# zju3dv/IntrinsicNeRF

Hardware: AMD Instinct MI355X
Metric: rays/sec (64+128 samples/ray) (higher is better)
Workload: dtype f32 (operands split into f16 hi+lo, 3 f16 MFMA products per MAC, fp32 accumulate); 1 GPU; Blender chair 800x800 frame (640000 rays), 64 coarse + 128 importance samples, coarse+fine intrinsic NeRF (D=8, W=256), white_bkgd, eval mode, default-init weights (seeds 0/1) with the density head calibrated so that acc spans (0, 1]; parallelism=ray-sharded x1, gather=none

## Files before the change

### intrinsicnerf_amd/_build.py

```python
import os
import shutil
import subprocess

PKG_DIR = os.path.dirname(os.path.abspath(__file__))
CSRC = os.path.join(PKG_DIR, "csrc")
LIB_PATH = os.path.join(PKG_DIR, "libinerf.so")
OBJ_DIR = os.path.join(CSRC, "_obj")
SOURCES = ["pack.cpp", "api.cpp", "mlp.hip", "mlp_f16.hip", "mlp_f16_t128.hip", "mlp_bwd.hip", "mlp_wgrad.hip", "train_api.hip", "ray_ops.hip", "frame_ops.hip", "cluster.hip", "cluster_fit.hip", "refresh.hip", "layered.hip", "losses.hip", "adam.hip", "batch.hip"]
HEADERS = [os.path.join(CSRC, "layout.h"), os.path.join(CSRC, "draws.h"), os.path.join(CSRC, "cluster_search.h"), os.path.join(CSRC, "mlp_common.h"), os.path.join(CSRC, "mlp_f16_dev.h"), os.path.join(CSRC, "mlp_f16_heads.h"), os.path.join(CSRC, "mlp_f16_pp.h"),
           os.path.join(os.path.dirname(PKG_DIR), "include", "inerf.h")]
FLAGS = ["--offload-arch=gfx950", "-O3", "-std=c++17", "-ffp-contract=off", "-fPIC", "-shared",
         "-Wno-comment", "-Wno-unused-result"]


EXTRA_FLAGS = {"mlp_bwd.hip": ["-mllvm", "-amdgpu-mfma-vgpr-form=1"]}
DIGEST_MARK = b"INERF_BUILD_DIGEST="


def source_digest():
    import hashlib
    h = hashlib.sha256()
    h.update(repr((SOURCES, FLAGS, sorted(EXTRA_FLAGS.items()))).encode())
    for path in [os.path.join(CSRC, s) for s in SOURCES] + HEADERS:
        h.update(os.path.basename(path).encode())
        with open(path, "rb") as fh:
            h.update(fh.read())
    return h.hexdigest()


def built_digest(lib_path=None):
    try:
        with open(lib_path or LIB_PATH, "rb") as fh:
            data = fh.read()
    except OSError:
        return ""
    i = data.find(DIGEST_MARK)
    return data[i + len(DIGEST_MARK): i + len(DIGEST_MARK) + 64].decode("ascii", "replace") if i >= 0 else ""


def _source_paths():
    return [os.path.join(CSRC, s) for s in SOURCES] + HEADERS


def sources_present():
    return all(os.path.exists(p) for p in _source_paths())


def _stale(lib_path=None):
    lib_path = lib_path or LIB_PATH
    if not os.path.exists(lib_path):
        return True
    csrc_paths = [p for p in _source_paths() if os.path.dirname(p) == CSRC]
    if not any(os.path.exists(p) for p in csrc_paths):
        return False
    present = [os.path.exists(p) for p in _source_paths()]
    if not all(present):
        missing = [os.path.relpath(p, os.path.dirname(CSRC)) for p, ok in zip(_source_paths(), present) if not ok]
        raise RuntimeError(f"intrinsicnerf_amd: the source tree is incomplete ({', '.join(missing)} missing): cannot tell whether "
                           f"{os.path.basename(lib_path)} was built from it.  Restore the files, or remove csrc/ and the headers entirely "
                           "for a binary deployment")
    return built_digest(lib_path) != source_digest()


def have_hipcc():
    return bool(shutil.which("hipcc")) or os.path.exists("/opt/rocm/bin/hipcc")


def build_library(force=False, verbose=False):
    if not force and not _stale():
        return LIB_PATH
    import fcntl
    with open(LIB_PATH + ".lock", "w") as lock:
        fcntl.flock(lock, fcntl.LOCK_EX)
        try:
            if not force and not _stale():
                return LIB_PATH
            hipcc = shutil.which("hipcc") or "/opt/rocm/bin/hipcc"
            if not os.path.exists(hipcc):
                raise RuntimeError("hipcc not found: cannot build libinerf.so (ROCm toolchain required)")
            os.makedirs(OBJ_DIR, exist_ok=True)
            import hashlib
            header_bytes = b"".join(open(h, "rb").read() for h in HEADERS)

            def compile_one(src):
                obj = os.path.join(OBJ_DIR, src + ".o")
                path = os.path.join(CSRC, src)
                flags = [f for f in FLAGS if f != "-shared"] + EXTRA_FLAGS.get(src, [])
                key = hashlib.sha256(repr(flags).encode() + open(path, "rb").read() + header_bytes).hexdigest()
                try:
                    cached = open(obj + ".key").read().strip()
                except OSError:
                    cached = ""
                if not force and os.path.exists(obj) and cached == key:
                    return obj, None
                cmd = [hipcc] + flags + ["-c", path, "-o", obj + f".{os.getpid()}.tmp"]
                if verbose:
                    print(" ".join(cmd))
                proc = subprocess.run(cmd, capture_output=True, text=True)
                if proc.returncode != 0:
                    return obj, proc.stdout + proc.stderr
                os.replace(obj + f".{os.getpid()}.tmp", obj)
                with open(obj + ".key", "w") as fh:
                    fh.write(key)
                return obj, None

            from concurrent.futures import ThreadPoolExecutor
            with ThreadPoolExecutor(max_workers=min(len(SOURCES), os.cpu_count() or 1)) as pool:
                results = list(pool.map(compile_one, SOURCES))
            errors = [e for _, e in results if e]
            if errors:
                raise RuntimeError("hipcc failed:\n" + "\n".join(errors))
            stamp_src = os.path.join(OBJ_DIR, f"build_digest.{os.getpid()}.cpp")
            with open(stamp_src, "w") as fh:
                fh.write('extern "C" const char* inerf_build_digest(void) { return "%s%s" + %d; }\n'
                         % (DIGEST_MARK.decode(), source_digest(), len(DIGEST_MARK)))
            tmp = f"{LIB_PATH}.{os.getpid()}.tmp"
            cmd = [hipcc, "--offload-arch=gfx950", "-shared", "-fPIC", "-x", "c++", stamp_src, "-x", "none"] + [o for o, _ in results] + ["-o", tmp]
            if verbose:
                print(" ".join(cmd))
            proc = subprocess.run(cmd, capture_output=True, text=True)
            os.remove(stamp_src)
            if proc.returncode != 0:
                raise RuntimeError("hipcc (link) failed:\n" + proc.stdout + proc.stderr)
            os.replace(tmp, LIB_PATH)
        finally:
            fcntl.flock(lock, fcntl.LOCK_UN)
    return LIB_PATH


if __name__ == "__main__":
    print(build_library(force=True, verbose=True))
```

### intrinsicnerf_amd/csrc/mlp_f16_dev.h

```cpp
#pragma once
#include <type_traits>

#include "mlp_common.h"

namespace inerf {

typedef float f32x4 __attribute__((ext_vector_type(4)));
typedef float f32x16 __attribute__((ext_vector_type(16)));
typedef _Float16 f16x8 __attribute__((ext_vector_type(8)));
typedef _Float16 f16x4 __attribute__((ext_vector_type(4)));
typedef unsigned int u32x4 __attribute__((ext_vector_type(4)));
typedef unsigned int u32x2 __attribute__((ext_vector_type(2)));

#ifndef INERF_WEIGHT_AUX
#define INERF_WEIGHT_AUX 0
#endif
struct WeightBuf {
    __amdgpu_buffer_rsrc_t rsrc;
    int voff;
    __device__ __forceinline__ f16x8 frag(int byte_off) const {
#ifdef INERF_ABL_WLOAD_L1
        byte_off &= 0xFFF;
#endif
        return __builtin_bit_cast(f16x8, __builtin_amdgcn_raw_buffer_load_b128(rsrc, voff, byte_off, INERF_WEIGHT_AUX));
    }
    __device__ __forceinline__ f32x4 vec4(int byte_off, int lane_bytes) const {
        return __builtin_bit_cast(f32x4, __builtin_amdgcn_raw_buffer_load_b128(rsrc, lane_bytes, byte_off, 0));
    }
    __device__ __forceinline__ float scalar(int byte_off) const {
        return __builtin_bit_cast(float, __builtin_amdgcn_raw_buffer_load_b32(rsrc, 0, byte_off, 0));
    }
};

#ifndef INERF_FRAG_AUX
#define INERF_FRAG_AUX 2
#endif
constexpr int kRowH = kColB + kWidth + 8;
constexpr int kPlaneH = kTilePoints * kRowH;
constexpr int kLdsBytesH = 2 * kPlaneH * 2;
constexpr float kF16Safe = 6.0e4f;

template <int PLANE = kPlaneH>
__device__ __forceinline__ void split_store(_Float16* hi_ptr, float v, float& amax) {
    const float t = v * kActScale;
    const _Float16 h = (_Float16)t;
    hi_ptr[0] = h;
    hi_ptr[PLANE] = (_Float16)(t - (float)h);
    amax = fmaxf(amax, fabsf(t));
}

template <int PLANE = kPlaneH>
__device__ __forceinline__ void hi_store_parked(_Float16* hi_ptr, float v, float& amax) {
    const float t = v * kActScale;
    const _Float16 h = (_Float16)t;
    hi_ptr[0] = h;
    hi_ptr[PLANE] = h;
    amax = fmaxf(amax, fabsf(t));
}

__device__ __forceinline__ void fast_sincosf(float a, float* sn, float* cs) {
    if (__builtin_expect(!(fabsf(a) < 32768.0f), 0)) { sincosf(a, sn, cs); return; }
    const float j = __builtin_rintf(a * 0.636619772367581343f);
    float r = __builtin_fmaf(-j, 1.5707963705062866f, a);
    r = __builtin_fmaf(-j, -4.371138828673793e-08f, r);
    r = __builtin_fmaf(-j, -1.7763568394002505e-15f, r);
    const float z = r * r;
    float sp = __builtin_fmaf(-1.9515295891e-4f, z, 8.3321608736e-3f);
    sp = __builtin_fmaf(sp, z, -1.6666654611e-1f);
    const float s = __builtin_fmaf(sp * z, r, r);
    float cp = __builtin_fmaf(2.443315711809948e-5f, z, -1.388731625493765e-3f);
    cp = __builtin_fmaf(cp, z, 4.166664568298827e-2f);
    const float c = __builtin_fmaf(cp * z, z, __builtin_fmaf(-0.5f, z, 1.0f));
    const int q = (int)j;
    const float ss = (q & 1) ? c : s, cc = (q & 1) ? s : c;
    *sn = (q & 2) ? -ss : ss;
    *cs = ((q + 1) & 2) ? -cc : cc;
}

#ifndef INERF_EPI_PKFMA
#define INERF_EPI_PKFMA 0
#endif
#ifndef INERF_GEMM_PRIO
#define INERF_GEMM_PRIO 1
#endif

template <int RB>
struct WidePreH {
    f16x8 w[2][RB][2];
    f32x4 b[RB][4];
    float inv;
};

template <int RB>
__device__ __forceinline__ void wide_prefetch_h(WidePreH<RB>& pre, const WeightBuf& wb, int frag_bytes ,
                                                int bias_bytes , int scale_bytes, int lane) {
    const int h16 = 16 * (lane >> 5);
#pragma unroll
    for (int kb = 0; kb < 2; ++kb)
#pragma unroll
        for (int rb = 0; rb < RB; ++rb)
#pragma unroll
            for (int part = 0; part < 2; ++part) pre.w[kb][rb][part] = wb.frag(frag_bytes + ((kb * RB + rb) * 2 + part) * 1024);
#pragma unroll
    for (int rb = 0; rb < RB; ++rb)
#pragma unroll
        for (int g = 0; g < 4; ++g) pre.b[rb][g] = wb.vec4(bias_bytes + (32 * rb + 8 * g) * 4, h16);
    pre.inv = wb.scalar(scale_bytes);
}

template <int RB, int KB0, int KB1, int ROW = kRowH, int PLANE = kPlaneH, bool ZERO = true, int KSTRIDE = RB * 2048, int PB = 2, int RBSTRIDE = 2048,
          bool PEEL = false, int NPROD = 3>
__device__ __forceinline__ void wide_gemm_h(const WidePreH<RB>& pre, const WeightBuf& wb, int frag_bytes,
                                            const _Float16* xl,
                                            int col0, int col1, int lane, f32x16 (&am)[RB][PB]) {
    constexpr int KBT = KB0 + KB1;
    static_assert(KBT % 2 == 0 && KBT >= 4, "k-block count");
    static_assert(PB == 2 || (PB == 1 && RB == 2) || (PB == 4 && RB == 1), "point blocks");
    static_assert(NPROD == 3 || (NPROD == 1 && PB == 4 && RB == 1), "the one-product form is the 128-point tile's");
    constexpr int NP = NPROD == 1 ? 1 : 2;
    if constexpr (ZERO && !PEEL) {
#pragma unroll
        for (int rb = 0; rb < RB; ++rb)
#pragma unroll
            for (int g = 0; g < 4; ++g)
#pragma unroll
                for (int i = 0; i < 4; ++i)
#pragma unroll
                    for (int pb = 0; pb < PB; ++pb) am[rb][pb][4 * g + i] = 0.0f;
    }
    const f32x16 zero_c = {0.0f, 0.0f, 0.0f, 0.0f, 0.0f, 0.0f, 0.0f, 0.0f, 0.0f, 0.0f, 0.0f, 0.0f, 0.0f, 0.0f, 0.0f, 0.0f};
    auto xoff = [&](int kb) { return kb < KB0 ? col0 + 16 * kb : col1 + 16 * (kb - KB0); };
    f16x8 w[4][RB][2], x[2][PB][2];
#pragma unroll
    for (int rb = 0; rb < RB; ++rb)
#pragma unroll
        for (int part = 0; part < NP; ++part) { w[0][rb][part] = pre.w[0][rb][part]; w[1][rb][part] = pre.w[1][rb][part]; }
#pragma unroll
    for (int pb = 0; pb < PB; ++pb)
#pragma unroll
        for (int part = 0; part < NP; ++part)
            x[0][pb][part] = *reinterpret_cast<const f16x8*>(xl + part * PLANE + xoff(0) + pb * 32 * ROW);
    int lo_off = PLANE;
    if constexpr (PEEL) asm volatile("" : "+v"(lo_off));
    const _Float16* xl_lo = xl + lo_off;

#define INERF_F16_STEP(K, I) INERF_F16_STEP_(K, I, false)
#define INERF_F16_STEP_(K, I, FIRST)                                                                                 \
    {                                                                                                                \
        const int k1_ = (K) + 1 < KBT ? (K) + 1 : KBT - 1;                                                           \
        const int k2_ = (K) + 2 < KBT ? (K) + 2 : KBT - 1;                                                           \
                                                                                    \
        const int xo_ = (KB1 == 0 && PEEL) ? col0 + 16 * ((K) + 1) : xoff(k1_);                                      \
        _Pragma("unroll") for (int rb = 0; rb < RB; ++rb)                                                            \
            _Pragma("unroll") for (int part = 0; part < NP; ++part)                                                  \
                w[((I) + 2) & 3][rb][part] = wb.frag(frag_bytes + k2_ * KSTRIDE + rb * RBSTRIDE + part * 1024);      \
        _Pragma("unroll") for (int pb = 0; pb < PB; ++pb)                                                            \
            _Pragma("unroll") for (int part = 0; part < NP; ++part)                                                  \
                x[((I) + 1) & 1][pb][part] =                                                                         \
                    *reinterpret_cast<const f16x8*>((PEEL && part ? xl_lo : xl + part * PLANE) + xo_ + pb * 32 * ROW); \
         \
        _Pragma("unroll") for (int rb = 0; rb < RB; ++rb)                                                            \
            _Pragma("unroll") for (int pb = 0; pb < PB; ++pb)                                                        \
                am[rb][pb] = __builtin_amdgcn_mfma_f32_32x32x16_f16(w[(I) & 3][rb][0], x[(I) & 1][pb][0], (FIRST) ? zero_c : am[rb][pb], 0, 0, 0); \
        if constexpr (NPROD == 3) {                                                                                  \
        _Pragma("unroll") for (int rb = 0; rb < RB; ++rb)                                                            \
            _Pragma("unroll") for (int pb = 0; pb < PB; ++pb)                                                        \
                am[rb][pb] = __builtin_amdgcn_mfma_f32_32x32x16_f16(w[(I) & 3][rb][0], x[(I) & 1][pb][1], am[rb][pb], 0, 0, 0); \
        _Pragma("unroll") for (int rb = 0; rb < RB; ++rb)                                                            \
            _Pragma("unroll") for (int pb = 0; pb < PB; ++pb)                                                        \
                am[rb][pb] = __builtin_amdgcn_mfma_f32_32x32x16_f16(w[(I) & 3][rb][1], x[(I) & 1][pb][0], am[rb][pb], 0, 0, 0); \
        }                                                                                                            \
         \
        if constexpr (NPROD == 1) {                                         \
            __builtin_amdgcn_sched_group_barrier(0x008, 1, 0);                                                       \
            __builtin_amdgcn_sched_group_barrier(0x100, 2, 0);                                                       \
            __builtin_amdgcn_sched_group_barrier(0x008, 1, 0);                                                       \
            __builtin_amdgcn_sched_group_barrier(0x100, 2, 0);                                                       \
            __builtin_amdgcn_sched_group_barrier(0x008, 1, 0);                                                       \
            __builtin_amdgcn_sched_group_barrier(0x020, 1, 0);                                                       \
            __builtin_amdgcn_sched_group_barrier(0x008, 1, 0);                                                       \
        } else if constexpr (PB == 4) {                                                                              \
            _Pragma("unroll") for (int q = 0; q < 2; ++q) {                                                         \
                __builtin_amdgcn_sched_group_barrier(0x008, 1, 0);                                                   \
                __builtin_amdgcn_sched_group_barrier(0x100, 2, 0);                                                   \
                __builtin_amdgcn_sched_group_barrier(0x008, 1, 0);                                                   \
                __builtin_amdgcn_sched_group_barrier(0x100, 2, 0);                                                   \
                __builtin_amdgcn_sched_group_barrier(0x008, 1, 0);                                                   \
            }                                                                                                        \
            __builtin_amdgcn_sched_group_barrier(0x008, 1, 0);                                                       \
            __builtin_amdgcn_sched_group_barrier(0x020, 1, 0);                                                       \
            __builtin_amdgcn_sched_group_barrier(0x008, 1, 0);                                                       \
            __builtin_amdgcn_sched_group_barrier(0x020, 1, 0);                                                       \
            __builtin_amdgcn_sched_group_barrier(0x008, 4, 0);                                                       \
        } else if constexpr (PB == 2) {                                                                              \
            _Pragma("unroll") for (int q = 0; q < 2 * RB; ++q) {                                                    \
                __builtin_amdgcn_sched_group_barrier(0x008, 1, 0);                                                   \
                __builtin_amdgcn_sched_group_barrier(0x020, 1, 0);                                                   \
                __builtin_amdgcn_sched_group_barrier(0x008, 1, 0);                                                   \
                __builtin_amdgcn_sched_group_barrier(0x100, 4 / (2 * RB), 0);                                        \
                __builtin_amdgcn_sched_group_barrier(0x008, 1, 0);                                                   \
            }                                                                                                        \
        } else {                                                                                                     \
            _Pragma("unroll") for (int q = 0; q < 2; ++q) {                                                         \
                __builtin_amdgcn_sched_group_barrier(0x008, 1, 0);                                                   \
                __builtin_amdgcn_sched_group_barrier(0x020, 1, 0);                                                   \
                __builtin_amdgcn_sched_group_barrier(0x008, 1, 0);                                                   \
                __builtin_amdgcn_sched_group_barrier(0x020, 1, 0);                                                   \
                __builtin_amdgcn_sched_group_barrier(0x008, 1, 0);                                                   \
                __builtin_amdgcn_sched_group_barrier(0x100, 1, 0);                                                   \
            }                                                                                                        \
        }                                                                                                            \
        __builtin_amdgcn_sched_barrier(0);                                                                           \
    }
    constexpr int KB4 = KBT & ~3;
#if INERF_GEMM_PRIO
    __builtin_amdgcn_s_setprio(INERF_GEMM_PRIO);
#endif
    if constexpr (PEEL) {
        static_assert(KB4 >= 4, "peeled k-blocks");
        INERF_F16_STEP_(0, 0, ZERO)
        INERF_F16_STEP(1, 1)
        INERF_F16_STEP(2, 2)
        INERF_F16_STEP(3, 3)
    }
#pragma unroll 1
    for (int kb = PEEL ? 4 : 0; kb < KB4; kb += 4) {
        INERF_F16_STEP(kb + 0, 0)
        INERF_F16_STEP(kb + 1, 1)
        INERF_F16_STEP(kb + 2, 2)
        INERF_F16_STEP(kb + 3, 3)
    }
    if constexpr (KBT - KB4 == 2) {
        INERF_F16_STEP(KB4 + 0, 0)
        INERF_F16_STEP(KB4 + 1, 1)
    }
#if INERF_GEMM_PRIO
    __builtin_amdgcn_s_setprio(0);
#endif
#undef INERF_F16_STEP
#undef INERF_F16_STEP_
}

typedef _Float16 f16x2 __attribute__((ext_vector_type(2)));

__device__ __forceinline__ float flag_f16_range(const MlpParams& p, int first_point, int tile_points, float amax, f16x2 amax2, int lane) {
    const float m = fmaxf(amax, fmaxf((float)amax2[0], (float)amax2[1]));
    if (p.status && __any(!(m <= kF16Safe)) && lane == 0) {
        int w0 = 0, w1 = 0;
        if (p.status_rays > 0) {
            int last = first_point + tile_points - 1;
            last = last < p.n_points ? last : p.n_points - 1;
            w0 = (p.ray0 + first_point / p.n_samples) / p.status_rays;
            w1 = (p.ray0 + last / p.n_samples) / p.status_rays;
        }
        for (int w = w0; w <= w1; ++w) atomicOr(p.status + w, INERF_STATUS_F16_RANGE);
    }
    return m;
}


__device__ __forceinline__ float split_upper_bound(float amax, f16x2 amax2) {
    const float h = fmaxf((float)amax2[0], (float)amax2[1]);
    const float a = amax > 0.0f ? __builtin_fmaf(amax, 0x1p-21f, amax) + 0x1p-25f : amax;
    const float b = h > 0.0f ? __builtin_fmaf(h, 0x1p-10f, h) + 0x1p-24f : h;
    return fmaxf(a, b);
}

__device__ __forceinline__ void pk_max3_into(f16x2& amax, f16x2 a, f16x2 b) {
#ifdef INERF_NO_MAX3
    amax = __builtin_elementwise_max(amax, __builtin_elementwise_max(a, b));
    return;
#endif
    unsigned m = __builtin_bit_cast(unsigned, amax);
    asm("v_pk_maximum3_f16 %0, %0, %1, %2" : "+v"(m) : "v"(__builtin_bit_cast(unsigned, a)), "v"(__builtin_bit_cast(unsigned, b)));
    amax = __builtin_bit_cast(f16x2, m);
}

__device__ __forceinline__ void split_pair(float t0, float t1, f16x2& hi, f16x2& lo) {
    const unsigned h = __builtin_bit_cast(unsigned, __builtin_amdgcn_cvt_pkrtz(t0, t1));
    unsigned l;
    asm("v_fma_mixlo_f16 %0, -%1, 1.0, %2 op_sel_hi:[1,0,0]" : "=v"(l) : "v"(h), "v"(t0));
    asm("v_fma_mixhi_f16 %0, -%1, 1.0, %2 op_sel:[1,0,0] op_sel_hi:[1,0,0]" : "+v"(l) : "v"(h), "v"(t1));
    hi = __builtin_bit_cast(f16x2, h);
    lo = __builtin_bit_cast(f16x2, l);
}

struct SaveDst {
    __amdgpu_buffer_rsrc_t rsrc;
    int voff;
    int stride;
};

struct Selector { f16x8 k[2]; };
__device__ __forceinline__ Selector plane_selector(int lane, float value = 1.0f) {
    Selector s;
#pragma unroll
    for (int kb = 0; kb < 2; ++kb)
#pragma unroll
        for (int i = 0; i < 8; ++i) s.k[kb][i] = (16 * kb + 8 * (lane >> 5) + i) == (lane & 31) ? (_Float16)value : (_Float16)0.0f;
    return s;
}
struct FragDst {
    __amdgpu_buffer_rsrc_t rsrc;
    unsigned voff;
};
template <int CBS = 8>
__device__ __forceinline__ unsigned frag_off(int kb, int cb, int plane) { return (unsigned)((kb * CBS + cb) * 2 + plane) * kFragBytes; }

template <int NB, int ROW, int PLANE, int CBS = 8>
__device__ __forceinline__ void planes_to_frag(const _Float16* xa ,
                                               const Selector& sel, const FragDst& dst) {
#ifdef INERF_ABL_NO_FRAG
    return;
#endif
    const f32x16 zero = {0.0f, 0.0f, 0.0f, 0.0f, 0.0f, 0.0f, 0.0f, 0.0f, 0.0f, 0.0f, 0.0f, 0.0f, 0.0f, 0.0f, 0.0f, 0.0f};
#pragma unroll
    for (int cb = 0; cb < NB; ++cb) {
        f16x8 ah[2][2], al[2][2];
#pragma unroll
        for (int pb = 0; pb < 2; ++pb) {
            const _Float16* src = xa + pb * 32 * ROW + 32 * cb;
            ah[pb][0] = *reinterpret_cast<const f16x8*>(src);          ah[pb][1] = *reinterpret_cast<const f16x8*>(src + 16);
            al[pb][0] = *reinterpret_cast<const f16x8*>(src + PLANE);  al[pb][1] = *reinterpret_cast<const f16x8*>(src + PLANE + 16);
        }
        f32x16 th[2], tl[2];
#pragma unroll
// ... 293 lines not shown
```

### intrinsicnerf_amd/csrc/mlp_f16_t128.hip

```cpp
#include <stdio.h>
#include <stdlib.h>

#include <type_traits>
#include <vector>

#include "mlp_f16_dev.h"
#include "mlp_f16_heads.h"
#include "mlp_f16_pp.h"

#ifndef INERF_T128_PEEL
#define INERF_T128_PEEL 1
#endif
#ifndef INERF_GATE_TRUNK_PARK
#define INERF_GATE_TRUNK_PARK 1
#endif

namespace inerf {

constexpr int kPtsT = 128;
constexpr int kPlaneT = kPtsT * kRowD;
constexpr int kLdsBytesT = 2 * kPlaneT * 2;
constexpr int kSemScratchBytesT = 8 * 2 * 16 * 64 * 4;

constexpr int kEncCacheBytesT = 2 * kPtsT * kEncCols * 2;
// ... 566 lines not shown
                        const _Float16* src = ldst + r * kRowD + 32 * wave + 16 * (lane_t >> 5);
                        const f16x8 f0 = *reinterpret_cast<const f16x8*>(src), f1 = *reinterpret_cast<const f16x8*>(src + 8);
                        bool bad = false;
#pragma unroll
                        for (int i = 0; i < 8; ++i) bad |= !(fabsf((float)f0[i]) <= kF16Safe) || !(fabsf((float)f1[i]) <= kF16Safe);
                        if (bad) pad_of(r)[0] = 1;
                    }
                }
                amax2 = f16x2{(_Float16)0.0f, (_Float16)0.0f};
            }
            f32x16 amv[1][2];
            f32x4 biasv[1][4];
            float invv;
            wide_gemm_h<1, 18, 0, kRowD, kPlaneT, true, 2048, 2, 2048, kPeel>(prev, wb, frag128(L.views, 18), xr_h, 0, 0, lane_t, amv);
            load_bias<1>(biasv, invv, wb, (L.views.b + 32 * cg) * 4, (L.views.b + kHalf) * 4, lane_t);
            if constexpr (kMode == kGateHeads) prefetch_w<2>(pre2, wb, frag256(L.as1, 16));
            else                               prefetch_w<1, 4096>(pre1, wb, frag32(L.trunk[0], 4));
            f16x8 hi[2][2], lo[2][2];
            to_operands<1, false, 2, !kSave>(amv, invv, biasv, amax2, hi, lo);
            if constexpr (kMode == kGateHeads) flag_operands(hi);
            if constexpr (kSave) {
                int lane_o = lane_t;
                asm volatile("" : "+v"(lane_o));
                FragDst d;
                d.rsrc = __builtin_amdgcn_make_buffer_rsrc(p.save + p.save_off[SAVE_VH], 0, (int)((unsigned)n_tiles64 * (unsigned)(kFragTileBytes / 2)), 0x00020000);
                d.voff = (unsigned)(2 * tile + ph) * (unsigned)(kFragTileBytes / 2) + (unsigned)cg * (2u * kFragBytes) + (unsigned)lane_o * 16u;
                operands_to_frag<1, 4>(hi, lo, accumulator_selector(lane_o), d);
            }
            regop_gemm<2>(wb, (L.resr.w + cg * 2 * 2 * 256) * 4, hi, lo, part_res);
        }
        __syncthreads();
        bool my_flagged = false;
        if constexpr (kMode == kGateHeads) {
            const u32x4 f = *reinterpret_cast<const u32x4*>(pad_of(16 * wave + (lane_t & 15)));
            my_flagged = (f[0] | f[1] | f[2] | f[3]) != 0u;
        }
        if (lane_t < 32) {
#pragma unroll
            for (int pb = 0; pb < 2; ++pb) {
                float* ex = reinterpret_cast<float*>(ldst + (lane_t + 32 * pb + 64 * ph) * kRowD + kColExD) + 8 * cg;
                *reinterpret_cast<f32x4*>(ex) = part_as[pb];
                *reinterpret_cast<f32x4*>(ex + 4) = part_res[pb];
            }
        }
        auto sem_ex = [&](int g, int r) {
            return reinterpret_cast<float*>(ldst) + (g < 2 ? 64 + 32 * g : kPlaneT / 2 + 32 * (g - 1)) + r * (kRowD / 2);
        };
        if constexpr (kSsr) {
            if (sem) {
#pragma unroll
                for (int pb = 0; pb < 2; ++pb) {
                    u32x4 sem_v[4];
#pragma unroll
                    for (int g = 0; g < 4; ++g) sem_v[g] = __builtin_amdgcn_raw_buffer_load_b128(sem_rsrc, sem_slot + (pb * 4 + g) * 1024, 0, 1);
#pragma unroll
                    for (int g = 0; g < 4; ++g)
                        *reinterpret_cast<u32x4*>(sem_ex(cg, 64 * ph + 32 * pb + (lane_t & 31)) + 8 * g + 4 * (lane_t >> 5)) = sem_v[g];
                }
            }
        }
        __syncthreads();
        if constexpr (kSsr) {
            if (sem) {
                const int r = 16 * wave + (lane_t & 15), c8 = 8 * (lane_t >> 4);
                f32x4 s0 = *reinterpret_cast<const f32x4*>(sem_ex(0, r) + c8), s1 = *reinterpret_cast<const f32x4*>(sem_ex(0, r) + c8 + 4);
#pragma unroll
                for (int g = 1; g < 4; ++g) {
                    s0 += *reinterpret_cast<const f32x4*>(sem_ex(g, r) + c8);
                    s1 += *reinterpret_cast<const f32x4*>(sem_ex(g, r) + c8 + 4);
                }
                const float sem_inv2 = wb.scalar((L.sem2.b + 16 * L.sem_rbs) * 4);
                const f32x4 b0 = wb.vec4((L.sem2.b + c8) * 4, 0), b1 = wb.vec4((L.sem2.b + c8 + 4) * 4, 0);
#pragma unroll
                for (int i = 0; i < 4; ++i) {
                    if (my_valid && c8 + i < p.n_classes) __builtin_nontemporal_store(__builtin_fmaf(s0[i], sem_inv2, b0[i]), out_row + INERF_BASE_CHANNELS + c8 + i);
                    if (my_valid && c8 + 4 + i < p.n_classes) __builtin_nontemporal_store(__builtin_fmaf(s1[i], sem_inv2, b1[i]), out_row + INERF_BASE_CHANNELS + c8 + 4 + i);
                }
            }
        }
        const bool whole_rows = kMode != kGateHeads && p.channels == INERF_BASE_CHANNELS && tile * kPtsT + kPtsT <= p.n_points &&
                                (reinterpret_cast<uintptr_t>(p.raw) & 15) == 0;
        auto stage_row = [&](int r) { return reinterpret_cast<float*>(ldst + kPlaneT + r * kRowD + 128); };
        if (lane_t < 16 && my_valid) {
            const float* ex = reinterpret_cast<const float*>(ldst + (16 * wave + lane_t) * kRowD + kColExD);
            f32x4 as4 = {0.0f, 0.0f, 0.0f, 0.0f}, res4 = {0.0f, 0.0f, 0.0f, 0.0f};
#pragma unroll
            for (int w = 0; w < 4; ++w) {
                as4 += *reinterpret_cast<const f32x4*>(ex + 8 * w);
                res4 += *reinterpret_cast<const f32x4*>(ex + 8 * w + 4);
            }
            const f32x4 b_as = wb.vec4(L.as2.b * 4, 0), b_res = wb.vec4(L.res.b * 4, 0);
            const float inv_as = wb.scalar((L.as2.b + 16) * 4), inv_res = wb.scalar((L.res.b + 16) * 4);
#pragma unroll
            for (int i = 0; i < 4; ++i) {
                as4[i] = __builtin_fmaf(as4[i], inv_as, b_as[i]);
                res4[i] = __builtin_fmaf(res4[i], inv_res, b_res[i]);
            }
            const float a0 = sigmoid_ref_h(as4[0]), a1 = sigmoid_ref_h(as4[1]), a2 = sigmoid_ref_h(as4[2]);
            const float sh = sigmoid_ref_h(as4[3]);
            const float r0 = sigmoid_ref_h(res4[0]), r1 = sigmoid_ref_h(res4[1]), r2 = sigmoid_ref_h(res4[2]);
            const float c0 = __fadd_rn(__fmul_rn(a0, sh), r0), c1 = __fadd_rn(__fmul_rn(a1, sh), r1), c2 = __fadd_rn(__fmul_rn(a2, sh), r2);
            if constexpr (kMode == kGateHeads) {
                const int pt = p.gate_idx[my_pt];
                float* const row = p.raw + (size_t)pt * p.channels;
                __builtin_nontemporal_store(c0, row + 0); __builtin_nontemporal_store(c1, row + 1); __builtin_nontemporal_store(c2, row + 2);
                __builtin_nontemporal_store(a0, row + 4); __builtin_nontemporal_store(a1, row + 5); __builtin_nontemporal_store(a2, row + 6);
                __builtin_nontemporal_store(sh, row + 7);
                __builtin_nontemporal_store(r0, row + 8); __builtin_nontemporal_store(r1, row + 9); __builtin_nontemporal_store(r2, row + 10);
                if (my_flagged && p.status)
                    atomicOr(p.status + (p.status_rays > 0 ? (p.ray0 + pt / p.n_samples) / p.status_rays : 0), INERF_STATUS_F16_RANGE);
            } else if (whole_rows) {
                float* st = stage_row(16 * wave + lane_t);
                *reinterpret_cast<f32x4*>(st) = f32x4{c0, c1, c2, sig4[0]};
                *reinterpret_cast<f32x4*>(st + 4) = f32x4{a0, a1, a2, sh};
                st[8] = r0; st[9] = r1; st[10] = r2;
            } else {
                __builtin_nontemporal_store(c0, out_row + 0);
                __builtin_nontemporal_store(c1, out_row + 1);
                __builtin_nontemporal_store(c2, out_row + 2);
                __builtin_nontemporal_store(sig4[0], out_row + 3);
                __builtin_nontemporal_store(a0, out_row + 4); __builtin_nontemporal_store(a1, out_row + 5); __builtin_nontemporal_store(a2, out_row + 6);
                __builtin_nontemporal_store(sh, out_row + 7);
                __builtin_nontemporal_store(r0, out_row + 8); __builtin_nontemporal_store(r1, out_row + 9); __builtin_nontemporal_store(r2, out_row + 10);
            }
        }
        if (whole_rows && lane_t < 44) {
            f32x4 v;
#pragma unroll
            for (int i = 0; i < 4; ++i) {
                const int e = 4 * lane_t + i, pt = e / INERF_BASE_CHANNELS;
                v[i] = stage_row(16 * wave + pt)[e - INERF_BASE_CHANNELS * pt];
            }
            __builtin_nontemporal_store(v, reinterpret_cast<f32x4*>(p.raw + (size_t)(tile * kPtsT + 16 * wave) * INERF_BASE_CHANNELS) + lane_t);
        }
        if constexpr (kMode != kGateHeads) flag_f16_range(p, tile * kPtsT, kPtsT, amax, amax2, lane_t);
    }
    if (kSave && p.act_max) {
        float m = split_upper_bound(amax, amax2) * (1.0f / kActScale);
#pragma unroll
        for (int o = 32; o > 0; o >>= 1) m = fmaxf(m, __shfl_xor(m, o));
        if (lane == 0 && m == m) atomicMax(reinterpret_cast<unsigned int*>(p.act_max), __builtin_bit_cast(unsigned int, m));
    }
}

template <bool kSsr, bool kSave = false, bool kPipe = false>
__global__ __launch_bounds__(512, 2) void k_encode_mlp_f16x3_t128(const MlpParams p) {
    encode_mlp_t128_tiles<kSsr, kSave, kPipe, kWhole>(p);
}
__global__ __launch_bounds__(512, 2) void k_mlp_gate_trunk_f16x3(const MlpParams p) { encode_mlp_t128_tiles<false, false, false, kGateTrunk>(p); }
__global__ __launch_bounds__(512, 2) void k_mlp_gate_heads_f16x3(const MlpParams p) { encode_mlp_t128_tiles<false, false, false, kGateHeads>(p); }
__global__ __launch_bounds__(512, 2) void k_mlp_gate_probe_f16(const MlpParams p) { encode_mlp_t128_tiles<false, false, false, kGateProbe>(p); }
__global__ __launch_bounds__(512, 2) void k_mlp_gate_trunk_listed_f16x3(const MlpParams p) { encode_mlp_t128_tiles<false, false, false, kGateTrunk, true>(p); }

static int64_t gate_budget_points() {
    int64_t bytes = (int64_t)2 << 30;
    if (const char* e = getenv("INERF_GATE_BYTES")) {
        const double v = atof(e);
        if (v >= 1.0) bytes = v < 6.0e10 ? (int64_t)v : (int64_t)6.0e10;
    }
    return bytes / (kGateRecordBytes + 4);
}

bool mlp_gate_applies(const inerf_net_desc& net, uint32_t flags) {
    return net.precision == INERF_PREC_F16X3 && net.variant == INERF_VARIANT_OBJECT && !(flags & INERF_FLAG_ENDPOINT) && !getenv("INERF_F16_KERNEL");
}

GatePlan mlp_gate_plan(int64_t n_rays, int n_samples) {
    GatePlan g{};
    if (n_rays <= 0 || n_samples < 1) return g;
    const int64_t fit = gate_budget_points() / n_samples;
    g.rays_per_sub = fit < 1 ? 1 : fit < n_rays ? fit : n_rays;
    g.n_sub = (n_rays + g.rays_per_sub - 1) / g.rays_per_sub;
    const int64_t pts = g.rays_per_sub * n_samples;
    auto up = [](int64_t b) { return (b + 255) / 256 * 256; };
    g.idx_off = up(pts * kGateRecordBytes);
    g.count_off = g.idx_off + up(pts * 4);
    g.cand_off = g.count_off + up(g.n_sub * 4);
    g.cand_count_off = g.cand_off + up(pts * 4);
    g.bytes = g.cand_count_off + up(g.n_sub * 4);
    return g;
}

int launch_mlp_f16x3_gated(const MlpParams& p0, int64_t n_rays, void* gate_ws, bool probe, hipStream_t stream) {
    const GatePlan g = mlp_gate_plan(n_rays, p0.n_samples);
    char* const ws = static_cast<char*>(gate_ws);
    unsigned int* const counts = reinterpret_cast<unsigned int*>(ws + g.count_off);
    unsigned int* const cand_counts = reinterpret_cast<unsigned int*>(ws + g.cand_count_off);
    hipError_t e = hipMemsetAsync(counts, 0, (size_t)g.n_sub * 4, stream);
    if (e == hipSuccess && probe) e = hipMemsetAsync(cand_counts, 0, (size_t)g.n_sub * 4, stream);
    if (e != hipSuccess) return record(e);
    static PerDeviceOnce attr_set;
    if (attr_set.first()) {
        e = hipFuncSetAttribute(reinterpret_cast<const void*>(k_mlp_gate_trunk_f16x3), hipFuncAttributeMaxDynamicSharedMemorySize, kLdsBytesTrunk);
        if (e == hipSuccess) e = hipFuncSetAttribute(reinterpret_cast<const void*>(k_mlp_gate_heads_f16x3), hipFuncAttributeMaxDynamicSharedMemorySize, kLdsBytesT);
        if (e == hipSuccess) e = hipFuncSetAttribute(reinterpret_cast<const void*>(k_mlp_gate_probe_f16), hipFuncAttributeMaxDynamicSharedMemorySize, kLdsBytesT);
        if (e == hipSuccess) e = hipFuncSetAttribute(reinterpret_cast<const void*>(k_mlp_gate_trunk_listed_f16x3), hipFuncAttributeMaxDynamicSharedMemorySize, kLdsBytesTrunk);
        if (e != hipSuccess) return record(e);
        attr_set.mark();
    }
    for (int64_t s = 0; s < g.n_sub; ++s) {
        const int64_t r0 = s * g.rays_per_sub, nr = n_rays - r0 < g.rays_per_sub ? n_rays - r0 : g.rays_per_sub;
        MlpParams p = p0;
        p.rays += r0 * INERF_RAY_FLOATS;
        p.z += r0 * p0.n_samples;
        p.raw += r0 * p0.n_samples * p0.channels;
        p.ray0 = (int)r0;
        p.n_points = (int)(nr * p0.n_samples);
        p.n_tiles = (p.n_points + kPtsT - 1) / kPtsT;
        p.gate_rec = reinterpret_cast<unsigned char*>(ws);
        p.gate_idx = reinterpret_cast<int*>(ws + g.idx_off);
        p.gate_count = counts + s;
        p.cand_idx = reinterpret_cast<int*>(ws + g.cand_off);
        p.cand_count = cand_counts + s;
        if (p.probe_out) p.probe_out = p0.probe_out + 2 * r0 * p0.n_samples;
        const int grid = p.n_tiles < device_cus() ? p.n_tiles : device_cus();
        if (probe) {
            hipLaunchKernelGGL(k_mlp_gate_probe_f16, dim3(grid), dim3(512), kLdsBytesT, stream, p);
            hipLaunchKernelGGL(k_mlp_gate_trunk_listed_f16x3, dim3(grid), dim3(512), kLdsBytesTrunk, stream, p);
        } else {
            hipLaunchKernelGGL(k_mlp_gate_trunk_f16x3, dim3(grid), dim3(512), kLdsBytesTrunk, stream, p);
        }
        hipLaunchKernelGGL(k_mlp_gate_heads_f16x3, dim3(grid), dim3(512), kLdsBytesT, stream, p);
    }
    e = hipGetLastError();
    if (e == hipSuccess && getenv("INERF_GATE_LOG")) {
        std::vector<unsigned int> h((size_t)g.n_sub), hc((size_t)g.n_sub, 0u);
        e = hipStreamSynchronize(stream);
        if (e == hipSuccess) e = hipMemcpy(h.data(), counts, h.size() * 4, hipMemcpyDeviceToHost);
        if (e == hipSuccess && probe) e = hipMemcpy(hc.data(), cand_counts, hc.size() * 4, hipMemcpyDeviceToHost);
        unsigned long long kept = 0, cand = 0;
        for (unsigned int c : h) kept += c;
        for (unsigned int c : hc) cand += c;
        const double pts = (double)(n_rays * p0.n_samples);
        fprintf(stderr, "inerf gate: %lld rays x %d samples in %lld sub-launches, %llu of %lld points survive (%.4f)", (long long)n_rays,
                p0.n_samples, (long long)g.n_sub, kept, (long long)(n_rays * p0.n_samples), (double)kept / pts);
        if (probe) fprintf(stderr, ", %llu are the probe's candidates (%.4f)", cand, (double)cand / pts);
        fprintf(stderr, "\n");
    }
    return record(e);
}

int launch_mlp_f16x3_t128(MlpParams& p, int64_t n_points, bool ssr, hipStream_t stream) {
    p.n_tiles = (int)((n_points + kPtsT - 1) / kPtsT);
    const int grid = p.n_tiles < device_cus() ? p.n_tiles : device_cus();
    const bool save = p.save != nullptr;
    if (ssr && save) return INERF_E_UNSUPPORTED;
    const char* form = getenv("INERF_F16_KERNEL");
    const bool pipe = !ssr && !save && form && form[0] == 'p';
    void (*kern)(const MlpParams) = ssr ? k_encode_mlp_f16x3_t128<true> : save ? k_encode_mlp_f16x3_t128<false, true>
                                  : pipe ? k_encode_mlp_f16x3_t128<false, false, true> : k_encode_mlp_f16x3_t128<false>;
    static PerDeviceOnce attr_sets[4];
    PerDeviceOnce& attr_set = attr_sets[ssr ? 1 : save ? 2 : pipe ? 3 : 0];
    if (attr_set.first()) {
        hipError_t e = hipFuncSetAttribute(reinterpret_cast<const void*>(kern), hipFuncAttributeMaxDynamicSharedMemorySize, kLdsBytesT);
        if (e != hipSuccess) return record(e);
        attr_set.mark();
    }
    hipLaunchKernelGGL(kern, dim3(grid), dim3(512), kLdsBytesT, stream, p);
    return record(hipGetLastError());
}

}
```

Baseline: 1.829 million rays/s.

## Add two-workgroup-per-CU gate probe kernel with 256-thread tiles

Adds a new probe kernel for the gated MLP path that runs 256-thread workgroups, two per CU. Each wave handles 64 output rows across all 128 points (RB=2, PB=4, one-product f16 MFMA), and the kernel carries its own MFMA/load interleave schedule. The host launches up to twice as many workgroups for the probe stage, and the old 512-thread probe stays available through an environment variable. The aim is better latency hiding and less barrier stall per workgroup in the probe pass, at the cost of more register pressure and duplicated LDS park buffers. This only matters when the probe path is taken.

```diff
diff --git a/intrinsicnerf_amd/_build.py b/intrinsicnerf_amd/_build.py
--- a/intrinsicnerf_amd/_build.py
+++ b/intrinsicnerf_amd/_build.py
@@ -7,7 +7,7 @@
 LIB_PATH = os.path.join(PKG_DIR, "libinerf.so")
 OBJ_DIR = os.path.join(CSRC, "_obj")
 SOURCES = ["pack.cpp", "api.cpp", "mlp.hip", "mlp_f16.hip", "mlp_f16_t128.hip", "mlp_bwd.hip", "mlp_wgrad.hip", "train_api.hip", "ray_ops.hip", "frame_ops.hip", "cluster.hip", "cluster_fit.hip", "refresh.hip", "layered.hip", "losses.hip", "adam.hip", "batch.hip"]
-HEADERS = [os.path.join(CSRC, "layout.h"), os.path.join(CSRC, "draws.h"), os.path.join(CSRC, "cluster_search.h"), os.path.join(CSRC, "mlp_common.h"), os.path.join(CSRC, "mlp_f16_dev.h"), os.path.join(CSRC, "mlp_f16_heads.h"), os.path.join(CSRC, "mlp_f16_pp.h"),
+HEADERS = [os.path.join(CSRC, "layout.h"), os.path.join(CSRC, "draws.h"), os.path.join(CSRC, "cluster_search.h"), os.path.join(CSRC, "mlp_common.h"), os.path.join(CSRC, "mlp_f16_dev.h"), os.path.join(CSRC, "mlp_f16_heads.h"), os.path.join(CSRC, "mlp_f16_pp.h"), os.path.join(CSRC, "mlp_f16_probe.h"),
            os.path.join(os.path.dirname(PKG_DIR), "include", "inerf.h")]
 FLAGS = ["--offload-arch=gfx950", "-O3", "-std=c++17", "-ffp-contract=off", "-fPIC", "-shared",
          "-Wno-comment", "-Wno-unused-result"]
diff --git a/intrinsicnerf_amd/csrc/mlp_f16_dev.h b/intrinsicnerf_amd/csrc/mlp_f16_dev.h
--- a/intrinsicnerf_amd/csrc/mlp_f16_dev.h
+++ b/intrinsicnerf_amd/csrc/mlp_f16_dev.h
@@ -115,8 +115,8 @@
                                             int col0, int col1, int lane, f32x16 (&am)[RB][PB]) {
     constexpr int KBT = KB0 + KB1;
     static_assert(KBT % 2 == 0 && KBT >= 4, "k-block count");
-    static_assert(PB == 2 || (PB == 1 && RB == 2) || (PB == 4 && RB == 1), "point blocks");
-    static_assert(NPROD == 3 || (NPROD == 1 && PB == 4 && RB == 1), "the one-product form is the 128-point tile's");
+    static_assert(PB == 2 || (PB == 1 && RB == 2) || (PB == 4 && RB == 1) || (PB == 4 && RB == 2 && NPROD == 1), "point blocks");
+    static_assert(NPROD == 3 || (NPROD == 1 && PB == 4 && (RB == 1 || RB == 2)), "the one-product form is the 128-point tile's");
     constexpr int NP = NPROD == 1 ? 1 : 2;
     if constexpr (ZERO && !PEEL) {
 #pragma unroll
@@ -171,7 +171,17 @@
                 am[rb][pb] = __builtin_amdgcn_mfma_f32_32x32x16_f16(w[(I) & 3][rb][1], x[(I) & 1][pb][0], am[rb][pb], 0, 0, 0); \
         }                                                                                                            \
          \
-        if constexpr (NPROD == 1) {                                         \
+        if constexpr (NPROD == 1 && RB == 2) {           \
+            _Pragma("unroll") for (int q = 0; q < 2; ++q) {                                                         \
+                __builtin_amdgcn_sched_group_barrier(0x008, 1, 0);                                                   \
+                __builtin_amdgcn_sched_group_barrier(0x100, 1, 0);                                                   \
+                __builtin_amdgcn_sched_group_barrier(0x008, 1, 0);                                                   \
+                __builtin_amdgcn_sched_group_barrier(0x100, 1, 0);                                                   \
+                __builtin_amdgcn_sched_group_barrier(0x008, 1, 0);                                                   \
+                __builtin_amdgcn_sched_group_barrier(0x020, 1, 0);                                                   \
+                __builtin_amdgcn_sched_group_barrier(0x008, 1, 0);                                                   \
+            }                                                                                                        \
+        } else if constexpr (NPROD == 1) {                                  \
             __builtin_amdgcn_sched_group_barrier(0x008, 1, 0);                                                       \
             __builtin_amdgcn_sched_group_barrier(0x100, 2, 0);                                                       \
             __builtin_amdgcn_sched_group_barrier(0x008, 1, 0);                                                       \
diff --git a/intrinsicnerf_amd/csrc/mlp_f16_probe.h b/intrinsicnerf_amd/csrc/mlp_f16_probe.h
--- /dev/null
+++ b/intrinsicnerf_amd/csrc/mlp_f16_probe.h
@@ -0,0 +1,186 @@
+#pragma once
+
+namespace inerf {
+
+constexpr int kProbeWg2Threads = 256;
+constexpr int kProbeWg2ExtBytes = kPtsT * kParkExtPieces * 16;
+constexpr int kLdsBytesProbeWg2 = kPlaneT * 2 + kProbeWg2ExtBytes;
+static_assert(2 * kLdsBytesProbeWg2 <= 160 * 1024, "two probe workgroups share the CU's LDS");
+
+__device__ __forceinline__ void mlp_gate_probe_wg2_tiles(const MlpParams& p) {
+    constexpr int kParts = kProbeWg2Threads / kPtsT;
+    extern __shared__ __attribute__((aligned(16))) _Float16 ldst[];
+    const int tid = threadIdx.x;
+    const int wave = __builtin_amdgcn_readfirstlane(tid >> 6);
+    const NetLayout& L = p.L;
+
+    _Float16* const xw = ldst + (tid & 31) * kRowD;
+    const _Float16* const xr = xw + 8 * ((tid & 63) >> 5);
+    _Float16* const xd = xw + 4 * ((tid & 63) >> 5) + 64 * wave;
+
+    WeightBuf wb;
+    wb.rsrc = __builtin_amdgcn_make_buffer_rsrc(const_cast<float*>(p.wts), 0, L.total_floats * 4, 0x00020000);
+    wb.voff = (tid & 63) * 16;
+    auto frag64 = [&](const GemmSlot& s, int kbt) { return (s.w + wave * kbt * 2 * 2 * 256) * 4; };
+    auto pad_of = [&](int r) { return reinterpret_cast<int*>(ldst + r * kRowD + kWidth + kDirCols); };
+
+    WidePreH<2> pre;
+    auto pf = [&](const GemmSlot& s, int kbt, int kb_first) { prefetch_w<2, 4096, 2048, 1>(pre, wb, frag64(s, kbt) + kb_first * 4096); };
+    pf(L.trunk[0], 4, 0);
+
+    for (int tile = blockIdx.x; tile < p.n_tiles; tile += gridDim.x) {
+        int lane_t = tid;
+        asm volatile("" : "+v"(lane_t));
+        lane_t &= 63;
+        float amax = 0.0f;
+        f16x2 amax2 = {(_Float16)0.0f, (_Float16)0.0f};
+        {
+            int tid_o = tid;
+            asm volatile("" : "+v"(tid_o));
+            const int pt = tid_o % kPtsT, part = tid_o / kPtsT;
+            int gp = tile * kPtsT + pt;
+            gp = gp < p.n_points ? gp : p.n_points - 1;
+            const int ray = gp / p.n_samples;
+            const float* __restrict__ r = p.rays + (size_t)ray * INERF_RAY_FLOATS;
+            _Float16* row = ldst + pt * kRowD;
+            const float zz = __builtin_nontemporal_load(p.z + gp);
+            float x[3];
+#pragma unroll
+            for (int c = 0; c < 3; ++c) x[c] = __fadd_rn(r[c], __fmul_rn(r[3 + c], zz));
+            auto hi_store = [&](_Float16* dst, float v) {
+                const float t = v * kActScale;
+                dst[0] = (_Float16)t;
+                amax = fmaxf(amax, fabsf(t));
+            };
+            for (int f = part; f < p.l_xyz; f += kParts) {
+                const float s = (float)(1 << f);
+#pragma unroll
+                for (int c = 0; c < 3; ++c) {
+                    float sn, cs;
+                    fast_sincosf(x[c] * s, &sn, &cs);
+                    hi_store(row + 3 + 6 * f + c, sn);
+                    hi_store(row + 6 + 6 * f + c, cs);
+                }
+            }
+            if (part == kParts - 1) {
+#pragma unroll
+                for (int c = 0; c < 3; ++c) hi_store(row + c, x[c]);
+                for (int c = 3 + 6 * p.l_xyz; c < kEncCols; ++c) row[c] = (_Float16)0.0f;
+            }
+        }
+        __syncthreads();
+        auto park_copy = [&](bool restore) {
+            int t = tid;
+            asm volatile("" : "+v"(t));
+            const int r = t >> 3, j = t & 7;
+            const bool in_row = j < kParkRowPieces;
+            _Float16* const cols = ldst + r * kRowD + j * 8;
+            _Float16* const parked = in_row ? cols + kColDirD : ldst + kPlaneT + (r * kParkExtPieces + (j - kParkRowPieces)) * 8;
+            u32x4 v[4];
+#pragma unroll
+            for (int i = 0; i < 4; ++i) {
+                const _Float16* const a = cols + i * 32 * kRowD;
+                const _Float16* const b = parked + (in_row ? i * 32 * kRowD : i * 32 * kParkExtPieces * 8);
+                v[i] = *reinterpret_cast<const u32x4*>(restore ? b : a);
+            }
+#pragma unroll
+            for (int i = 0; i < 4; ++i) {
+                _Float16* const a = cols + i * 32 * kRowD;
+                _Float16* const b = parked + (in_row ? i * 32 * kRowD : i * 32 * kParkExtPieces * 8);
+                *reinterpret_cast<u32x4*>(restore ? a : b) = v[i];
+            }
+        };
+        park_copy(false);
+
+        f32x16 am[2][4];
+        f32x4 bias[2][4];
+        float inv;
+        auto store_hi = [&](const GemmSlot& s, const GemmSlot& next, int kbt, int kb_first) {
+            load_bias<2>(bias, inv, wb, (s.b + 64 * wave) * 4, (s.b + kWidth) * 4, lane_t);
+            pf(next, kbt, kb_first);
+            __syncthreads();
+            wide_store_h<2, kRowD, kPlaneT, false, false, 4, true, true>(am, inv, bias, xd, true, amax2, nullptr, 0, 0, 0);
+            __syncthreads();
+        };
+        wide_gemm_h<2, 4, 0, kRowD, kPlaneT, true, 4096, 4, 2048, true, 1>(pre, wb, frag64(L.trunk[0], 4), xr, 0, 0, lane_t, am);
+        store_hi(L.trunk[0], L.trunk[1], 16, 0);
+#pragma unroll 1
+        for (int layer = 1; layer < kSkipInput; ++layer) {
+            wide_gemm_h<2, 16, 0, kRowD, kPlaneT, true, 4096, 4, 2048, true, 1>(pre, wb, frag64(L.trunk[layer], 16), xr, 0, 0, lane_t, am);
+            if (layer + 1 < kSkipInput) store_hi(L.trunk[layer], L.trunk[layer + 1], 16, 0);
+            else                        store_hi(L.trunk[layer], L.trunk[kSkipInput], 20, 4);
+        }
+        {
+            const GemmSlot& s = L.trunk[kSkipInput];
+            wide_gemm_h<2, 16, 0, kRowD, kPlaneT, true, 4096, 4, 2048, true, 1>(pre, wb, frag64(s, 20) + 4 * 4096, xr, 0, 0, lane_t, am);
+            pf(s, 20, 0);
+            __syncthreads();
+            park_copy(true);
+            __syncthreads();
+            wide_gemm_h<2, 4, 0, kRowD, kPlaneT, false, 4096, 4, 2048, false, 1>(pre, wb, frag64(s, 20), xr, 0, 0, lane_t, am);
+            store_hi(s, L.trunk[6], 16, 0);
+        }
+        wide_gemm_h<2, 16, 0, kRowD, kPlaneT, true, 4096, 4, 2048, true, 1>(pre, wb, frag64(L.trunk[6], 16), xr, 0, 0, lane_t, am);
+        store_hi(L.trunk[6], L.trunk[7], 16, 0);
+        wide_gemm_h<2, 16, 0, kRowD, kPlaneT, true, 4096, 4, 2048, true, 1>(pre, wb, frag64(L.trunk[7], 16), xr, 0, 0, lane_t, am);
+        store_hi(L.trunk[7], L.trunk[0], 4, 0);
+
+        bool keep[2];
+        unsigned kept[2];
+#pragma unroll
+        for (int h = 0; h < 2; ++h) {
+            const int pt16 = tile * kPtsT + 32 * wave + 16 * h;
+            const _Float16* const xs_g = ldst + (32 * wave + 16 * h + (lane_t & 15)) * kRowD + 8 * (lane_t >> 4);
+            float sigma, scale;
+            skinny_probe_h<8>(wb, L.alpha.w * 4, L.alpha.b * 4, (L.alpha.b + 16) * 4, xs_g, lane_t, sigma, scale);
+            const bool valid = lane_t < 16 && pt16 + lane_t < p.n_points;
+            keep[h] = valid && !(sigma < -kProbeKappa * scale);
+            kept[h] = __builtin_amdgcn_readfirstlane((unsigned)__ballot(keep[h]));
+            float piece[4];
+#pragma unroll
+            for (int i = 0; i < 4; ++i) {
+                const int e = 4 * (lane_t < 44 ? lane_t : 43) + i, pt = e / INERF_BASE_CHANNELS;
+                const float s_pt = __shfl(sigma, pt);
+                piece[i] = e - INERF_BASE_CHANNELS * pt == 3 ? s_pt : 0.0f;
+            }
+            if (p.channels == INERF_BASE_CHANNELS && pt16 + 16 <= p.n_points && (reinterpret_cast<uintptr_t>(p.raw) & 15) == 0) {
+                if (lane_t < 44)
+                    __builtin_nontemporal_store(f32x4{piece[0], piece[1], piece[2], piece[3]},
+                                                reinterpret_cast<f32x4*>(p.raw + (size_t)pt16 * INERF_BASE_CHANNELS) + lane_t);
+            } else if (valid) {
+                float* const out_row = p.raw + (size_t)(pt16 + lane_t) * p.channels;
+#pragma unroll
+                for (int c = 0; c < INERF_BASE_CHANNELS; ++c) __builtin_nontemporal_store(c == 3 ? sigma : 0.0f, out_row + c);
+            }
+            if (p.probe_out && valid) {
+                p.probe_out[2 * (size_t)(pt16 + lane_t)] = sigma;
+                p.probe_out[2 * (size_t)(pt16 + lane_t) + 1] = scale;
+            }
+        }
+        if (lane_t == 0) {
+            pad_of(2 * wave)[0] = __popc(kept[0]);
+            pad_of(2 * wave + 1)[0] = __popc(kept[1]);
+        }
+        __syncthreads();
+        int before = 0, total = 0;
+#pragma unroll
+        for (int g = 0; g < 8; ++g) {
+            const int c = pad_of(g)[0];
+            total += c;
+            before += g < 2 * wave ? c : 0;
+        }
+        if (tid == 0) pad_of(8)[0] = total > 0 ? (int)atomicAdd(p.cand_count, (unsigned)total) : 0;
+        __syncthreads();
+        const int slot0 = __builtin_amdgcn_readfirstlane(pad_of(8)[0] + before);
+        const int slot1 = slot0 + __popc(kept[0]);
+        const int pt32 = tile * kPtsT + 32 * wave;
+        if (keep[0]) p.cand_idx[slot0 + __popc(kept[0] & ((1u << lane_t) - 1u))] = pt32 + lane_t;
+        if (keep[1]) p.cand_idx[slot1 + __popc(kept[1] & ((1u << lane_t) - 1u))] = pt32 + 16 + lane_t;
+        flag_f16_range(p, tile * kPtsT, kPtsT, amax, amax2, lane_t);
+        __syncthreads();
+    }
+}
+
+__global__ __launch_bounds__(kProbeWg2Threads, 2) void k_mlp_gate_probe_wg2_f16(const MlpParams p) { mlp_gate_probe_wg2_tiles(p); }
+
+}
diff --git a/intrinsicnerf_amd/csrc/mlp_f16_t128.hip b/intrinsicnerf_amd/csrc/mlp_f16_t128.hip
--- a/intrinsicnerf_amd/csrc/mlp_f16_t128.hip
+++ b/intrinsicnerf_amd/csrc/mlp_f16_t128.hip
@@ -742,6 +742,10 @@
 __global__ __launch_bounds__(512, 2) void k_mlp_gate_probe_f16(const MlpParams p) { encode_mlp_t128_tiles<false, false, false, kGateProbe>(p); }
 __global__ __launch_bounds__(512, 2) void k_mlp_gate_trunk_listed_f16x3(const MlpParams p) { encode_mlp_t128_tiles<false, false, false, kGateTrunk, true>(p); }
 
+}
+#include "mlp_f16_probe.h"
+namespace inerf {
+
 static int64_t gate_budget_points() {
     int64_t bytes = (int64_t)2 << 30;
     if (const char* e = getenv("INERF_GATE_BYTES")) {
@@ -785,9 +789,12 @@
         if (e == hipSuccess) e = hipFuncSetAttribute(reinterpret_cast<const void*>(k_mlp_gate_heads_f16x3), hipFuncAttributeMaxDynamicSharedMemorySize, kLdsBytesT);
         if (e == hipSuccess) e = hipFuncSetAttribute(reinterpret_cast<const void*>(k_mlp_gate_probe_f16), hipFuncAttributeMaxDynamicSharedMemorySize, kLdsBytesT);
         if (e == hipSuccess) e = hipFuncSetAttribute(reinterpret_cast<const void*>(k_mlp_gate_trunk_listed_f16x3), hipFuncAttributeMaxDynamicSharedMemorySize, kLdsBytesTrunk);
+        if (e == hipSuccess) e = hipFuncSetAttribute(reinterpret_cast<const void*>(k_mlp_gate_probe_wg2_f16), hipFuncAttributeMaxDynamicSharedMemorySize, kLdsBytesProbeWg2);
         if (e != hipSuccess) return record(e);
         attr_set.mark();
     }
+    const char* const wg_env = getenv("INERF_PROBE_WG");
+    const bool probe_wg2 = !(wg_env && wg_env[0] == '1');
     for (int64_t s = 0; s < g.n_sub; ++s) {
         const int64_t r0 = s * g.rays_per_sub, nr = n_rays - r0 < g.rays_per_sub ? n_rays - r0 : g.rays_per_sub;
         MlpParams p = p0;
@@ -805,7 +812,12 @@
         if (p.probe_out) p.probe_out = p0.probe_out + 2 * r0 * p0.n_samples;
         const int grid = p.n_tiles < device_cus() ? p.n_tiles : device_cus();
         if (probe) {
-            hipLaunchKernelGGL(k_mlp_gate_probe_f16, dim3(grid), dim3(512), kLdsBytesT, stream, p);
+            if (probe_wg2) {
+                const int grid2 = p.n_tiles < 2 * device_cus() ? p.n_tiles : 2 * device_cus();
+                hipLaunchKernelGGL(k_mlp_gate_probe_wg2_f16, dim3(grid2), dim3(kProbeWg2Threads), kLdsBytesProbeWg2, stream, p);
+            } else {
+                hipLaunchKernelGGL(k_mlp_gate_probe_f16, dim3(grid), dim3(512), kLdsBytesT, stream, p);
+            }
             hipLaunchKernelGGL(k_mlp_gate_trunk_listed_f16x3, dim3(grid), dim3(512), kLdsBytesTrunk, stream, p);
         } else {
             hipLaunchKernelGGL(k_mlp_gate_trunk_f16x3, dim3(grid), dim3(512), kLdsBytesTrunk, stream, p);
```

New measurement: 1.920 million rays/s, median of 6. 1.05x the previous value.
